# jstmn/cppflow

Hardware: AMD Instinct MI355X
Metric: LM-IK iterations/sec (seeds x waypoints) (higher is better)
Workload: dtype f32

## Files before the change

cppflow_amd/csrc/cppflow_hip.hip:

```cpp
#include <hip/hip_runtime.h>

#include <dlfcn.h>

#include <atomic>
#include <cmath>
#include <cstdio>
#include <cstring>
#include <mutex>
#include <new>
#include <string>
#include <type_traits>
#include <vector>

#include "../../include/cppflow_hip_debug.h"
#include "lmik_device.h"
#include "robots_gen.h"

using namespace cppf;

namespace cppf {
bool launch_fused_static(int static_id, int coll, unsigned grid, size_t lds, hipStream_t st, const FusedArgs& args);
int fused_static_block();
}

// ... 397 lines not shown
    if (const char* dump = std::getenv("CPPF_RTC_DUMP")) {
        std::ofstream f(dump);
        f << source;
    }
    uint64_t key = fnv1a(source);
    for (int i = 0; i < kEmbeddedCount; ++i) key = fnv1a(kEmbeddedSources[i], key);
    for (int i = 0; i < kRtcOptionCount; ++i) key = fnv1a(kRtcOptions[i], key);
    key = fnv1a(rtc_version_string(), key);
    char hex[32];
    std::snprintf(hex, sizeof hex, "%016llx", (unsigned long long)key);
    const std::string dir = rtc_cache_dir(cache_dir), file = dir + "/robot_" + hex + ".cppfrtc";
    std::vector<std::string> names;
    std::string code;
    if (!rtc_cache_read(dir, file, names, code)) {
        if (int rc = rtc_compile(source, with_quad, names, code)) return rc;
        rtc_cache_write(dir, file, names, code);
    }
    DeviceGuard device_guard__(robot->device);
    if (device_guard__.err != hipSuccess)
        return fail(CPPF_ERR_HIP, std::string("cppflow_hip: selecting the robot's device failed: ") + hipGetErrorString(device_guard__.err));
    RtcModule* m = new (std::nothrow) RtcModule();
    if (!m) return fail(CPPF_ERR_HIP, "cppflow_hip: out of host memory");
    hipError_t e = hipModuleLoadData(&m->module, code.data());
    for (int i = 0; e == hipSuccess && i < RTC_COUNT; ++i) {
        if (!with_quad && (i == RTC_QUAD0 || i == RTC_QUAD1)) continue;
        e = hipModuleGetFunction(&m->fn[i], m->module, names[(size_t)i].c_str());
    }
    if (e != hipSuccess) {
        if (m->module) (void)hipModuleUnload(m->module);
        delete m;
        return fail(CPPF_ERR_HIP, std::string("cppflow_hip: loading the specialised code object failed: ") + hipGetErrorString(e));
    }
    robot->rtc = m;
    return CPPF_OK;
}

int cppf_robot_ndof(const cppf_robot* robot) { return robot ? robot->desc.ndof : CPPF_ERR_INVALID; }

int cppf_debug_fused_single_offset(void) { return (int)__builtin_offsetof(FusedArgs, single); }

int cppf_debug_rtc_compile(const cppf_robot_desc* desc, const char* cache_dir) {
    cppf_robot* rb = nullptr;
    if (int rc = cppf_robot_create(desc, kNoDevice, &rb)) return rc;
    rb->static_id = -1;
    rb->device = kNoDevice;
    const int rc = cppf_robot_specialize(rb, cache_dir);
    delete rb;
    return rc;
}

int cppf_robot_specialization(const cppf_robot* robot) {
    if (!robot) return CPPF_ERR_INVALID;
    return robot->static_id >= 0 ? robot->static_id : (robot->rtc ? CPPF_SPECIALIZATION_RTC : -1);
}

int cppf_debug_set(cppf_robot* robot, int key, int value) {
    CPPF_REQUIRE(robot, "robot handle is NULL");
    CPPF_REQUIRE(key >= 0 && key < CPPF_TUNE_COUNT, "unknown tuning key");
    robot->tune[key].store(value == CPPF_TUNE_DEFAULT ? kTuneDefaults[key] : value, std::memory_order_relaxed);
    return CPPF_OK;
}

int cppf_debug_get(const cppf_robot* robot, int key, int* value) {
    CPPF_REQUIRE(robot && value, "robot / value is NULL");
    CPPF_REQUIRE(key >= 0 && key < CPPF_TUNE_COUNT, "unknown tuning key");
    *value = tune(robot, key);
    return CPPF_OK;
}

int cppf_set_obstacles(cppf_robot* robot, int n_obs, const float* cuboids, const float* Rt) {
    CPPF_REQUIRE(robot, "robot handle is NULL");
    CPPF_REQUIRE(n_obs >= 0 && n_obs <= CPPF_MAX_OBSTACLES, "n_obs out of range");
    CPPF_REQUIRE(n_obs == 0 || (cuboids && Rt), "cuboids / Rt is NULL");
    for (int o = 0; o < n_obs; ++o) {
        const float* R = Rt + o * 12;
        const float I[9] = {1, 0, 0, 0, 1, 0, 0, 0, 1};
        for (int k = 0; k < 9; ++k)
            CPPF_REQUIRE(std::fabs(R[k] - I[k]) < 1e-8f, "only axis-aligned cuboids are supported (R must be I)");
        for (int k = 0; k < 3; ++k) {
            CPPF_REQUIRE(cuboids[o * 6 + k] <= cuboids[o * 6 + 3 + k], "cuboid min corner > max corner");
            robot->coll.obs_lo[o][k] = R[9 + k] + cuboids[o * 6 + k];
            robot->coll.obs_hi[o][k] = R[9 + k] + cuboids[o * 6 + 3 + k];
        }
    }
    robot->coll.nobs = n_obs;
    return CPPF_OK;
}

int cppf_set_joint_limit_padding(cppf_robot* robot, const float* lo_padded, const float* hi_padded) {
    CPPF_REQUIRE(robot, "robot handle is NULL");
    if (!lo_padded || !hi_padded) {
        robot->coll.has_jl = 0;
        return CPPF_OK;
    }
    for (int j = 0; j < robot->desc.ndof; ++j) {
        robot->coll.jl_lo[j] = lo_padded[j];
        robot->coll.jl_hi[j] = hi_padded[j];
    }
    robot->coll.has_jl = 1;
    return CPPF_OK;
}

int cppf_forward_kinematics(const cppf_robot* robot, const float* x, int n, float* poses, void* stream) {
    CPPF_ENTER(robot);
    CPPF_REQUIRE(n >= 0, "n < 0");
    if (n == 0) return CPPF_OK;
    CPPF_REQUIRE(x && poses, "x / poses is NULL");
    hipStream_t st = (hipStream_t)stream;
    return for_ndof(robot->desc.ndof, [&](auto dof) {
        hipLaunchKernelGGL((fk_kernel<decltype(dof)::D>), dim3(grid_for(n)), dim3(kBlock), 0, st, robot->chain, robot->coll, n, x, poses);
        return check_launch();
    });
}

int cppf_jacobian(const cppf_robot* robot, const float* x, int n, float* J, void* stream) {
    CPPF_ENTER(robot);
    CPPF_REQUIRE(n >= 0, "n < 0");
    if (n == 0) return CPPF_OK;
    CPPF_REQUIRE(x && J, "x / J is NULL");
    hipStream_t st = (hipStream_t)stream;
    return for_ndof(robot->desc.ndof, [&](auto dof) {
        hipLaunchKernelGGL((jacobian_kernel<decltype(dof)::D>), dim3(grid_for(n)), dim3(kBlock), 0, st, robot->chain, robot->coll, n, x, J);
        return check_launch();
    });
}

int cppf_pose_errors(const cppf_robot* robot, const float* x, const float* target, int S, int W, float* e,
                     float* current_poses, void* stream) {
    CPPF_ENTER(robot);
    CPPF_REQUIRE(S >= 0 && W >= 0, "S / W < 0");
    const size_t n = (size_t)S * W;
    if (n == 0) return CPPF_OK;
    CPPF_REQUIRE(n <= 0x7fffffffu, "S*W exceeds 2^31-1 rows");
    CPPF_REQUIRE(x && target, "x / target is NULL");
    hipStream_t st = (hipStream_t)stream;
    return for_ndof(robot->desc.ndof, [&](auto dof) {
        hipLaunchKernelGGL((pose_errors_kernel<decltype(dof)::D>), dim3(grid_for(n)), dim3(kBlock), 0, st, robot->chain, robot->coll,
                           (int)n, W, x, target, e, current_poses);
        return check_launch();
    });
}

int cppf_clamp_to_joint_limits(const cppf_robot* robot, float* x, int n, void* stream) {
    CPPF_ENTER(robot);
    CPPF_REQUIRE(n >= 0, "n < 0");
    if (n == 0) return CPPF_OK;
    CPPF_REQUIRE(x, "x is NULL");
    const size_t total = (size_t)n * robot->desc.ndof;
    hipLaunchKernelGGL(clamp_kernel, dim3(grid_for(total)), dim3(kBlock), 0, (hipStream_t)stream, robot->chain, total, x);
    return check_launch();
}

}

namespace {

int make_lm_kernel_params(const cppf_robot* robot, const cppf_lm_params* params, LmK& prm) {
    CPPF_REQUIRE(params, "params is NULL");
    CPPF_REQUIRE(params->n_steps >= 1, "n_steps must be >= 1");
    CPPF_REQUIRE(params->clamp == 1 || params->n_steps == 1, "clamp = 0 is only defined for a single step");
    CPPF_REQUIRE(params->lm_lambda > 0.f, "lm_lambda must be > 0");
    CPPF_REQUIRE(params->alpha_position > 0.f && params->alpha_rotation > 0.f, "alpha_position / alpha_rotation must be > 0");
    CPPF_REQUIRE(params->solver == CPPF_SOLVER_AUTO || params->solver == CPPF_SOLVER_F32 || params->solver == CPPF_SOLVER_F64,
                 "unknown solver");
    CPPF_REQUIRE(params->solver_gate >= 0.f, "solver_gate must be >= 0 (0 = the default tolerance)");
    CPPF_REQUIRE(params->shape == CPPF_SHAPE_AUTO || params->shape == CPPF_SHAPE_ROW || params->shape == CPPF_SHAPE_QUAD,
// ... 1048 lines not shown
```

cppflow_amd/csrc/kernels_chain.h:

```cpp
#pragma once


template <int D>
__device__ __forceinline__ void load_x(const float* __restrict__ x, size_t row, float (&q)[D]) {
    const float* p = x + row * D;
    if constexpr (D % 4 == 0) {
#pragma unroll
        for (int k = 0; k < D / 4; ++k) {
            const float4 v = reinterpret_cast<const float4*>(p)[k];
            q[4 * k] = v.x, q[4 * k + 1] = v.y, q[4 * k + 2] = v.z, q[4 * k + 3] = v.w;
        }
    } else {
#pragma unroll
        for (int j = 0; j < D; ++j) q[j] = p[j];
    }
}

template <int D>
__device__ __forceinline__ void store_x(float* __restrict__ x, size_t row, const float (&q)[D]) {
    float* p = x + row * D;
    if constexpr (D % 4 == 0) {
#pragma unroll
        for (int k = 0; k < D / 4; ++k)
            reinterpret_cast<float4*>(p)[k] = make_float4(q[4 * k], q[4 * k + 1], q[4 * k + 2], q[4 * k + 3]);
// ... 86 lines not shown
}

#ifndef CPPF_LEAN_TRIG
#define CPPF_LEAN_TRIG 1
#endif
#ifndef CPPF_LEAN_RPY_FAST
#define CPPF_LEAN_RPY_FAST 1
#endif
__device__ __forceinline__ float atan_lean_poly(float a) {
    const float s = a * a;
    float p = 0.007374001666903496f;
    p = CPPF_FMA(p, s, -0.03551986813545227f);
    p = CPPF_FMA(p, s, 0.08216774463653564f);
    p = CPPF_FMA(p, s, -0.13398799300193787f);
    p = CPPF_FMA(p, s, 0.1986185610294342f);
    p = CPPF_FMA(p, s, -0.3332539498806f);
    return CPPF_FMA(a * s, p, a);
}
__device__ __forceinline__ float atan_lean_fixup(float a, float ax, float ay, float x, float y) {
    float r = atan_lean_poly(a);
    r = ay > ax ? 1.57079632679489661923f - r : r;
    r = x < 0.f ? 3.14159265358979323846f - r : r;
    return __builtin_copysignf(r, y);
}
__device__ __forceinline__ void atan2_pair_lean(float y1, float x1, float y2, float x2, float& r1, float& r2) {
    const float ax1 = fabsf(x1), ay1 = fabsf(y1), ax2 = fabsf(x2), ay2 = fabsf(y2);
    const float mx1 = fmaxf(fmaxf(ax1, ay1), 1e-15f), mx2 = fmaxf(fmaxf(ax2, ay2), 1e-15f);
    const float inv = __builtin_amdgcn_rcpf(mx1 * mx2);
    r1 = atan_lean_fixup(fminf(ax1, ay1) * (inv * mx2), ax1, ay1, x1, y1);
    r2 = atan_lean_fixup(fminf(ax2, ay2) * (inv * mx1), ax2, ay2, x2, y2);
}
__device__ __forceinline__ float asin_lean(float x) {
    const float ax = fabsf(x);
    const bool big = ax > 0.5f;

    const float z = big ? CPPF_FMA(-0.5f, ax, 0.5f) : x * x;
    const float t = big ? __builtin_amdgcn_sqrtf(z) : ax;
    float p = 0.05158697068691254f;
    p = CPPF_FMA(p, z, 0.03919339179992676f);
    p = CPPF_FMA(p, z, 0.07554031163454056f);
    p = CPPF_FMA(p, z, 0.16664926707744598f);
    float r = CPPF_FMA(t * z, p, t);
    r = big ? CPPF_FMA(-2.f, r, 1.57079632679489661923f) : r;
    return __builtin_copysignf(r, x);
}

template <bool LEAN = false>
__device__ __forceinline__ void pose_error(const float (&Rt)[9], const float (&tt)[3], const float (&R)[9],
                                           const float (&p)[3], float (&e)[6]) {
    const float e20 = dot3(Rt[6], Rt[7], Rt[8], R[0], R[1], R[2]);
    const float e21 = dot3(Rt[6], Rt[7], Rt[8], R[3], R[4], R[5]);
    const float e22 = dot3(Rt[6], Rt[7], Rt[8], R[6], R[7], R[8]);
    const float e10 = dot3(Rt[3], Rt[4], Rt[5], R[0], R[1], R[2]);
    const float e00 = dot3(Rt[0], Rt[1], Rt[2], R[0], R[1], R[2]);
    float sp = -e20;
    sp = sp > 1.f ? 1.f : (sp < -1.f ? -1.f : sp);
    if constexpr (LEAN && CPPF_LEAN_TRIG != 0) {
        const bool general = !(fabsf(sp) <= 0.5f) | !(fabsf(e21) <= e22) | !(fabsf(e10) <= e00);
        if (CPPF_LEAN_RPY_FAST != 0 && __builtin_expect(__builtin_amdgcn_ballot_w64(general) == 0ull, 1)) {
            const float inv = __builtin_amdgcn_rcpf(e22 * e00);
            const float a1 = e21 * (inv * e00), a2 = e10 * (inv * e22);
            e[0] = atan_lean_poly(a1);
            e[2] = atan_lean_poly(a2);
            const float z = sp * sp;
            float p = 0.05158697068691254f;
            p = CPPF_FMA(p, z, 0.03919339179992676f);
            p = CPPF_FMA(p, z, 0.07554031163454056f);
            p = CPPF_FMA(p, z, 0.16664926707744598f);
            e[1] = CPPF_FMA(sp * z, p, sp);
        } else {
            atan2_pair_lean(e21, e22, e10, e00, e[0], e[2]);
            e[1] = asin_lean(sp);
        }
    } else {
        e[0] = atan2_lm(e21, e22);
        e[1] = asin_lm(sp);
        e[2] = atan2_lm(e10, e00);
    }
    e[3] = tt[0] - p[0];
    e[4] = tt[1] - p[1];
    e[5] = tt[2] - p[2];
}

__device__ __forceinline__ void pose_metrics(const float (&Rt)[9], const float (&tt)[3], const float (&R)[9],
                                             const float (&p)[3], float& pos_err, float& rot_err) {
    const float dx = tt[0] - p[0], dy = tt[1] - p[1], dz = tt[2] - p[2];
    pos_err = __builtin_sqrtf(CPPF_FMA(dz, dz, CPPF_FMA(dy, dy, dx * dx)));
    float E[9];
#pragma unroll
    for (int i = 0; i < 3; ++i)
#pragma unroll
        for (int j = 0; j < 3; ++j)
            E[3 * i + j] = dot3(Rt[3 * i], Rt[3 * i + 1], Rt[3 * i + 2], R[3 * j], R[3 * j + 1], R[3 * j + 2]);
    const float a0 = E[7] - E[5], a1 = E[2] - E[6], a2 = E[3] - E[1];
    const float sn = 0.5f * __builtin_sqrtf(CPPF_FMA(a2, a2, CPPF_FMA(a1, a1, a0 * a0)));
    const float cs = 0.5f * (E[0] + E[4] + E[8] - 1.f);
    const float theta = atan2f(sn, cs);
    rot_err = fmaxf(theta, 8.94427191e-4f);
}

template <int D>
__device__ __forceinline__ void lm_dual_solve_y(const float (&J)[6][D], const float (&e)[6], float lam_r, float lam_p,
                                                float (&y)[6], float& est) {
    float L[6][6], inv[6], dmax = 0.f;
#pragma unroll
    for (int j = 0; j < 6; ++j) {
        const float lam = j < 3 ? lam_r : lam_p;
#pragma unroll
        for (int i = j; i < 6; ++i) {
            float s = (i == j) ? lam : 0.f;
#pragma unroll
            for (int k = 0; k < D; ++k) s = cfma2(J[i][k], J[j][k], s);
            if (i == j) dmax = fmaxf(dmax, s);
#pragma unroll
            for (int k = 0; k < j; ++k) s = CPPF_FMA(-L[i][k], L[j][k], s);
            if (i == j) {
                s = fmaxf(s, lam);
                inv[j] = __builtin_amdgcn_rsqf(s);
            } else {
                L[i][j] = s * inv[j];
            }
        }
    }
#pragma unroll
    for (int i = 0; i < 6; ++i) {
        float s = e[i];
#pragma unroll
        for (int k = 0; k < i; ++k) s = CPPF_FMA(-L[i][k], y[k], s);
        y[i] = s * inv[i];
    }
#pragma unroll
    for (int i = 5; i >= 0; --i) {
        float s = y[i];
#pragma unroll
        for (int k = i + 1; k < 6; ++k) s = CPPF_FMA(-L[k][i], y[k], s);
        y[i] = s * inv[i];
    }
    est = dmax * fmaxf(fmaxf(fmaxf(fabsf(y[0]), fabsf(y[1])), fmaxf(fabsf(y[2]), fabsf(y[3]))), fmaxf(fabsf(y[4]), fabsf(y[5])));
}

#ifndef CPPF_LEAN_BLOCK_SOLVE
#define CPPF_LEAN_BLOCK_SOLVE 1
#endif
template <int D>
__device__ __forceinline__ void lm_dual_solve_y_blk(const float (&J)[6][D], const float (&e)[6], float lam_r, float lam_p,
                                                    float (&y)[6], float& est) {
    float A[6][6], dmax = 0.f;
#pragma unroll
    for (int i = 0; i < 6; ++i)
#pragma unroll
        for (int j = 0; j <= i; ++j) {
            float s = (i == j) ? (i < 3 ? lam_r : lam_p) : 0.f;
#pragma unroll
            for (int k = 0; k < D; ++k) s = cfma2(J[i][k], J[j][k], s);
            A[i][j] = s;
            if (i == j) dmax = fmaxf(dmax, s);
        }
    float w0[6][3], w1[6][3], ia[3], ib[3], ic[3];
#pragma unroll
    for (int k = 0; k < 3; ++k) {
        const int p = 2 * k;
        const float a = A[p][p], b = A[p + 1][p], c = A[p + 1][p + 1];
        const float det = fmaxf(CPPF_FMA(a, c, -(b * b)), (p + 1 < 3 ? lam_r : lam_p) * a);
        const float r = __builtin_amdgcn_rcpf(det);
        ia[k] = c * r, ib[k] = -(b * r), ic[k] = a * r;
#pragma unroll
        for (int i = p + 2; i < 6; ++i) {
            w0[i][k] = CPPF_FMA(A[i][p + 1], ib[k], A[i][p] * ia[k]);
            w1[i][k] = CPPF_FMA(A[i][p + 1], ic[k], A[i][p] * ib[k]);
        }
#pragma unroll
        for (int i = p + 2; i < 6; ++i)
#pragma unroll
            for (int j = p + 2; j <= i; ++j) A[i][j] = CPPF_FMA(-w1[i][k], A[j][p + 1], CPPF_FMA(-w0[i][k], A[j][p], A[i][j]));
    }
    float u[6];
#pragma unroll
    for (int i = 0; i < 6; ++i) u[i] = e[i];
#pragma unroll
    for (int k = 0; k < 3; ++k) {
        const int p = 2 * k;
// ... 288 lines not shown
```

cppflow_amd/csrc/kernels_collision.h:

```cpp
#pragma once

struct CollOut {
    float min_self, min_env;
    int self_hit, env_hit;
};

__device__ __forceinline__ bool cull_far(float lower2, float cull2) {
    return __builtin_amdgcn_ballot_w64(!(lower2 > cull2)) == 0ull;
}

__device__ __forceinline__ float mid_dist2(const float (&a)[3], const float (&b)[3]) {
    const float dx = a[0] - b[0], dy = a[1] - b[1], dz = a[2] - b[2];
    return CPPF_FMA(dz, dz, CPPF_FMA(dy, dy, dx * dx));
}

__device__ __forceinline__ float point_box_dist2(const float (&m)[3], const float* __restrict__ lo,
                                                 const float* __restrict__ hi) {
    const float ex = m[0] - clampf(m[0], lo[0], hi[0]), ey = m[1] - clampf(m[1], lo[1], hi[1]),
                ez = m[2] - clampf(m[2], lo[2], hi[2]);
    return CPPF_FMA(ez, ez, CPPF_FMA(ey, ey, ex * ex));
}

template <class RB>
__device__ __forceinline__ void fk_capsules_to_lds(const RB& rb, const CollK& co, const float (&q)[RB::D],
                                                   float* __restrict__ lds, int tid, float (&R)[9], float (&p)[3]) {
    frame_identity(R, p);
    for (int c = co.cap_begin[0]; c < co.cap_begin[1]; ++c) {
#pragma unroll
        for (int k = 0; k < 3; ++k) {
            lds[(c * 6 + k) * kBlock + tid] = co.cap_c[c][k];
            lds[(c * 6 + 3 + k) * kBlock + tid] = co.cap_h[c][k];
        }
    }
#pragma unroll
    for (int j = 0; j < RB::D; ++j) {
        fk_fixed_joint(rb, j, R, p);
        fk_joint(R, p, rb.pris(j), q[j]);
        for (int c = co.cap_begin[j + 1]; c < co.cap_begin[j + 2]; ++c) {
            float wc[3], wh[3];
            xform_point(R, p, co.cap_c[c][0], co.cap_c[c][1], co.cap_c[c][2], wc);
            xform_dir(R, co.cap_h[c][0], co.cap_h[c][1], co.cap_h[c][2], wh);
#pragma unroll
            for (int k = 0; k < 3; ++k) {
                lds[(c * 6 + k) * kBlock + tid] = wc[k];
                lds[(c * 6 + 3 + k) * kBlock + tid] = wh[k];
            }
        }
    }
}

template <class RB>
__device__ __forceinline__ void capsule_fk_static(const RB& rb, const float (&q)[RB::D], float (&R)[9], float (&p)[3],
                                                  float (&wc)[(RB::Table::L > 0 ? RB::Table::L : 1)][3],
                                                  float (&wh)[(RB::Table::L > 0 ? RB::Table::L : 1)][3]) {
    using T = typename RB::Table;
    frame_identity(R, p);
#pragma unroll
    for (int c = 0; c < T::L; ++c) {
        if (T::cap_link[c] < 0) {
#pragma unroll
            for (int k = 0; k < 3; ++k) {
                wc[c][k] = T::cap_c[c][k];
                wh[c][k] = T::cap_h[c][k];
            }
        }
    }
#pragma unroll
    for (int j = 0; j < RB::D; ++j) {
        fk_fixed_joint(rb, j, R, p);
        fk_joint(R, p, rb.pris(j), q[j]);
#pragma unroll
        for (int c = 0; c < T::L; ++c) {
            if (T::cap_link[c] == j) {
                xform_point(R, p, T::cap_c[c][0], T::cap_c[c][1], T::cap_c[c][2], wc[c]);
                xform_dir(R, T::cap_h[c][0], T::cap_h[c][1], T::cap_h[c][2], wh[c]);
            }
        }
    }
}

__device__ __forceinline__ uint32_t cuboids_in_reach(const CollK& co, const float (&c)[3], float cull2) {
    uint32_t near = 0u;
    for (int o = 0; o < co.nobs; ++o)
        if (!cull_far(point_box_dist2(c, co.obs_lo[o], co.obs_hi[o]), cull2)) near |= 1u << o;
    return near;
}

template <class RB, bool WANT_MIN>
__device__ __forceinline__ CollOut collide_tests_static(const CollK& co,
                                                        const float (&wc)[(RB::Table::L > 0 ? RB::Table::L : 1)][3],
                                                        const float (&wh)[(RB::Table::L > 0 ? RB::Table::L : 1)][3],
                                                        bool do_self, bool do_env) {
    using T = typename RB::Table;
    CollOut r;
    r.min_self = INFINITY;
    r.self_hit = 0;
    if (do_self) {
#pragma unroll
        for (int pi = 0; pi < T::P; ++pi) {
            const int a = T::pair_a[pi], b = T::pair_b[pi];
            if constexpr (!WANT_MIN) {
                if (cull_far(mid_dist2(wc[a], wc[b]), T::pair_cull[pi])) continue;
            }
            const float d2 = seg_seg_dist2(wc[a], wh[a], wc[b], wh[b], T::cap_a[a], T::cap_ia[a], T::cap_a[b], T::cap_ia[b]);
            if constexpr (WANT_MIN) {
                const float v = __builtin_sqrtf(d2) - (T::cap_r[a] + T::cap_r[b]);
                r.min_self = v < r.min_self ? v : r.min_self;
            } else {
                r.self_hit |= d2 < T::pair_thr[pi];
            }
        }
    }
    if constexpr (WANT_MIN) r.self_hit = r.min_self < 0.f;
    r.min_env = INFINITY;
    r.env_hit = 0;
    if (do_env) {
#pragma unroll
        for (int c = 0; c < T::L; ++c) {
            uint32_t near = ~0u;
            if constexpr (!WANT_MIN) {
                near = cuboids_in_reach(co, wc[c], T::cap_cull[c]);
                if (near == 0u) continue;
            }
            for (int o = 0; o < co.nobs; ++o) {
                if (!((near >> o) & 1u)) continue;
                const float d2 = seg_box_dist2(wc[c], wh[c], co.obs_lo[o], co.obs_hi[o]);
                if constexpr (WANT_MIN) {
                    const float v = __builtin_sqrtf(d2) - T::cap_r[c];
                    r.min_env = v < r.min_env ? v : r.min_env;
                } else {
                    r.env_hit |= d2 < T::cap_thr[c];
                }
            }
        }
        if constexpr (WANT_MIN) r.env_hit = r.min_env < 0.f;
    }
    return r;
}

__device__ __forceinline__ void lds_capsule(const float* __restrict__ lds, int tid, int c, float (&wc)[3], float (&wh)[3]) {
#pragma unroll
    for (int k = 0; k < 3; ++k) {
        wc[k] = lds[(c * 6 + k) * kBlock + tid];
        wh[k] = lds[(c * 6 + 3 + k) * kBlock + tid];
    }
}

template <bool WANT_MIN>
__device__ __forceinline__ CollOut collide_from_lds(const CollK& co, const float* __restrict__ lds, int tid,
                                                    bool do_self, bool do_env) {
    CollOut r;
    r.min_self = INFINITY;
    r.self_hit = 0;
    if (do_self) {
        for (int pi = 0; pi < co.npairs; ++pi) {
            const int a = co.pair_a[pi], b = co.pair_b[pi];
            float ca[3], ha[3], cb[3], hb[3];
            lds_capsule(lds, tid, a, ca, ha);
            lds_capsule(lds, tid, b, cb, hb);
            if constexpr (!WANT_MIN) {
                if (cull_far(mid_dist2(ca, cb), co.pair_cull[pi])) continue;
            }
            const float d2 = seg_seg_dist2(ca, ha, cb, hb, co.cap_a[a], co.cap_ia[a], co.cap_a[b], co.cap_ia[b]);
            if constexpr (WANT_MIN) {
// ... 70 lines not shown
```

cppflow_amd/csrc/kernels_fused.h:

```cpp
#pragma once


__device__ __forceinline__ void load_target(const float* __restrict__ target, int w, float (&Rt)[9], float (&tt)[3]) {
    const float* t = target + (size_t)w * 7;
    tt[0] = t[0], tt[1] = t[1], tt[2] = t[2];
    quat_to_mat(t[3], t[4], t[5], t[6], Rt);
}

struct RowSummary {
    float pos_err = 0.f, rot_err = 0.f, cost = 0.f;
    int self_hit = 0, env_hit = 0, jl = 0;
};

template <int CTRL>
__device__ __forceinline__ float dpp_or_zero(float x) {
    return __builtin_bit_cast(float, __builtin_amdgcn_update_dpp(0, __builtin_bit_cast(int, x), CTRL, 0xf, 0xf, false));
}

template <bool IS_MAX>
__device__ __forceinline__ float wave_reduce_to_lane63(float v) {
    auto op = [](float a, float b) { return IS_MAX ? fmaxf(a, b) : a + b; };
    const float s1 = dpp_or_zero<0x111>(v), s2 = dpp_or_zero<0x112>(v), s3 = dpp_or_zero<0x113>(v);
    v = op(op(v, s1), op(s2, s3));
    v = op(v, dpp_or_zero<0x114>(v));
    v = op(v, dpp_or_zero<0x118>(v));
    v = op(v, dpp_or_zero<0x142>(v));
    v = op(v, dpp_or_zero<0x143>(v));
    return v;
}

__device__ __forceinline__ void lds_barrier() { asm volatile("s_waitcnt lgkmcnt(0)\n\ts_barrier" ::: "memory"); }

template <class RB>
__device__ __forceinline__ void block_seed_summary(const RB& rb, int W, size_t row, bool active, const float (&q)[RB::D],
                                                   const RowSummary& rs, float* __restrict__ out) {
    constexpr int D = RB::D;
    __shared__ float s_q[kBlock / 64][D];
    __shared__ float s_red[kBlock / 64][8];
    const int tid = threadIdx.x, lane = tid & 63, wave = tid >> 6;
    const float rad2deg = 57.29577951308232087680f;
    const int wps = W >> 6;
    if (wps > 1) {
        if (lane == 0) {
#pragma unroll
            for (int j = 0; j < D; ++j) s_q[wave][j] = q[j];
        }
        lds_barrier();
    }
    const bool seed_ends_here = ((wave + 1) & (wps - 1)) == 0;
    const bool has_next = active && !(lane == 63 && seed_ends_here);
    const int nw = wave + 1 < kBlock / 64 ? wave + 1 : wave;
    float mrev = 0.f, mpri = 0.f;
    float dq[D], wr[D];
#pragma unroll
    for (int j = 0; j < D; ++j) {
        float qn = dpp_or_zero<0x130>(q[j]);
        qn = (lane == 63) ? s_q[nw][j] : qn;
        dq[j] = wr[j] = qn - q[j];
    }
    wrap_pi_all<D>(wr);
#pragma unroll
    for (int j = 0; j < D; ++j) {
        const bool pr = rb.pris(j);
        const float a = nan_to_inf(pr ? fabsf(100.f * dq[j]) : fabsf(rad2deg * wr[j]));
        mpri = fmaxf(mpri, pr ? a : 0.f);
        mrev = fmaxf(mrev, pr ? 0.f : a);
    }
    float v[8] = {nan_to_inf(100.f * rs.pos_err), nan_to_inf(rad2deg * rs.rot_err), has_next ? mrev : 0.f, has_next ? mpri : 0.f,
                  (float)rs.self_hit, (float)rs.env_hit, (float)rs.jl, rs.cost};
#pragma unroll
    for (int k = 0; k < 8; ++k) v[k] = active ? v[k] : 0.f;
#pragma unroll
    for (int k = 0; k < 4; ++k) v[k] = wave_reduce_to_lane63<true>(v[k]);
#pragma unroll
    for (int k = 4; k < 8; ++k) v[k] = wave_reduce_to_lane63<false>(v[k]);
    float* o = out + ((uint32_t)row >> (31 - __builtin_clz((uint32_t)W))) * 8;
    if (wps == 1) {
        if (active && lane == 63) {
#pragma unroll
            for (int k = 0; k < 8; ++k) o[k] = v[k];
        }
        return;
    }
    if (lane == 63) {
#pragma unroll
        for (int k = 0; k < 8; ++k) s_red[wave][k] = v[k];
    }
    lds_barrier();
    if (active && lane == 63 && seed_ends_here) {
        for (int i = 1; i < wps; ++i) {
#pragma unroll
            for (int k = 0; k < 4; ++k) v[k] = fmaxf(v[k], s_red[wave - i][k]);
#pragma unroll
            for (int k = 4; k < 8; ++k) v[k] += s_red[wave - i][k];
        }
#pragma unroll
        for (int k = 0; k < 8; ++k) o[k] = v[k];
    }
}

#ifndef CPPF_LM_PACE
#define CPPF_LM_PACE 1
#endif
__device__ __forceinline__ void lm_pace(uint32_t t0, int k, int pace) {
    if (CPPF_LM_PACE == 0 || pace == 0) return;
    const int lag = (int)((uint32_t)__builtin_amdgcn_s_memrealtime() - t0) - k * pace, half = pace >> 1;
    if (lag > half)
        __builtin_amdgcn_s_setprio(3);
    else if (lag > 0)
        __builtin_amdgcn_s_setprio(2);
    else if (lag > -half)
        __builtin_amdgcn_s_setprio(1);
    else
        __builtin_amdgcn_s_setprio(0);
}

template <class RB>
__device__ __forceinline__ void lm_row_load(int W, const float* __restrict__ x_in, const float* __restrict__ target,
                                            size_t row, float (&q)[RB::D], float (&Rt)[9], float (&tt)[3]) {
    load_x<RB::D>(x_in, row, q);
    load_target(target, (int)((uint32_t)row % (uint32_t)W), Rt, tt);
}

#ifndef CPPF_LEAD_SINCOS
#define CPPF_LEAD_SINCOS 2
#endif
#ifndef CPPF_FIRST_LEAN
#define CPPF_FIRST_LEAN 1
#endif
template <class RB, bool LEAD, bool FIRST = false>
constexpr int lead_sincos() {
    return LEAD ? (FIRST && CPPF_LEAD_SINCOS == 2 ? 3 : CPPF_LEAD_SINCOS) : 0;
}
template <class RB, bool LEAD, bool FIRST = false>
__device__ __forceinline__ bool lm_row_iterate(const RB& rb, const LmK& prm, const cppf_lm_outputs& out, size_t row, bool last,
                                               const float (&Rt)[9], const float (&tt)[3], float* __restrict__ gate_lds,
                                               float (&q)[RB::D]) {
    constexpr int D = RB::D;
    float delta[D];
    bool conv = false;
    {
        float R[9], p[3], ax[D][3], og[D][3], J[6][D], e[6];
        fk_ee_axes<RB, lead_sincos<RB, LEAD, FIRST>()>(rb, q, R, p, ax, og);
        pose_error<LEAD>(Rt, tt, R, p, e);
        if constexpr (!LEAD) {
            if (prm.tol_pos2 > 0.f) {
                conv = dot3(e[3], e[4], e[5], e[3], e[4], e[5]) < prm.tol_pos2 && dot3(e[0], e[1], e[2], e[0], e[1], e[2]) < prm.tol_rot2;
                if (__builtin_amdgcn_ballot_w64(!conv) == 0ull) return true;
            }
        }
        jacobian_from_axes<RB>(rb, p, ax, og, J);
        float est = 0.f;
        if constexpr (D < 6) {
            lm_primal_solve<D>(J, e, prm.lm_lambda, prm.a_pos, prm.a_rot, delta);
        } else {
            float y[6];
            if constexpr (LEAD && CPPF_LEAN_BLOCK_SOLVE != 0)
                lm_dual_solve_y_blk<D>(J, e, prm.lam_r, prm.lam_p, y, est);
// ... 27 lines not shown
                        cut |= (v < rb.lo(j)) | (v > rb.hi(j));
                    }
                    flag = flag && !cut;
                }
                if constexpr (LEAD) {
                    if (prm.gate_thr > -INFINITY) {
                        const float es2 = CPPF_FMA(prm.a_pos * prm.a_pos, dot3(e[3], e[4], e[5], e[3], e[4], e[5]),
                                                   prm.a_rot * prm.a_rot * dot3(e[0], e[1], e[2], e[0], e[1], e[2]));
                        flag = flag && est * est > prm.gate_rel2 * es2;
                    }
                }
                unsigned long long todo = __builtin_amdgcn_ballot_w64(flag);
                if (todo != 0ull) {
                    int rank = lm_gate_hand_over<D>(J, e, todo, gate_lds, flag);
                    lm_gate_solve<D>(prm.lam_r_d, prm.lam_p_d, todo, rank, gate_lds, flag, delta);
                    while ((todo = __builtin_amdgcn_ballot_w64(flag)) != 0ull) {
                        float R2[9], p2[3], ax2[D][3], og2[D][3], J2[6][D], e2[6];
#pragma unroll
                        for (int j = 0; j < D; ++j) asm volatile("" : "+v"(q[j]));
                        fk_ee_axes<RB, lead_sincos<RB, LEAD, FIRST>()>(rb, q, R2, p2, ax2, og2);
                        pose_error<LEAD>(Rt, tt, R2, p2, e2);
                        jacobian_from_axes<RB>(rb, p2, ax2, og2, J2);
                        rank = lm_gate_hand_over<D>(J2, e2, todo, gate_lds, flag);
                        lm_gate_solve<D>(prm.lam_r_d, prm.lam_p_d, todo, rank, gate_lds, flag, delta);
                    }
                }
            }
        }
    }
    if constexpr (!LEAD) {
        if (prm.tol_pos2 > 0.f) {
            if (!conv) {
#pragma unroll
                for (int j = 0; j < D; ++j) q[j] += delta[j];
                if (prm.clamp) clamp_row<RB>(rb, q);
            }
            return conv;
        }
    }
#pragma unroll
    for (int j = 0; j < D; ++j) q[j] += delta[j];
    if (prm.clamp) clamp_row<RB>(rb, q);
    return false;
}

template <class RB, int COLL>
__device__ __forceinline__ void lm_row_finish(const RB& rb, const CollK& co, const cppf_lm_outputs& out, float* lds, int tid,
                                              size_t row, const float (&Rt)[9], const float (&tt)[3], const float (&q)[RB::D],
                                              RowSummary& rs) {
    constexpr int D = RB::D;
    if (out.x_out) store_x<D>(out.x_out, row, q);
    const bool want_metrics = out.pos_err_m || out.rot_err_rad || out.seed_summary;
    if constexpr (COLL != 0) {
        const bool do_self = out.self_mask || out.min_self || out.ext_cost || out.seed_summary;
        const bool do_env = out.env_mask || out.min_env || out.ext_cost || out.seed_summary;
        rs.jl = jlim_hit<D>(co, q);
        CollOut c;
        auto metrics = [&](float (&R)[9], float (&p)[3]) {
            if (want_metrics) {
                fk_fixed_ee(rb, R, p);
                pose_metrics(Rt, tt, R, p, rs.pos_err, rs.rot_err);
                if (out.pos_err_m) out.pos_err_m[row] = rs.pos_err;
                if (out.rot_err_rad) out.rot_err_rad[row] = rs.rot_err;
            }
        };
        if constexpr (RB::kStatic) {
            constexpr int L = RB::Table::L > 0 ? RB::Table::L : 1;
            float wc[L][3], wh[L][3];
            {
                float R[9], p[3];
                capsule_fk_static<RB>(rb, q, R, p, wc, wh);
                metrics(R, p);
            }
            c = collide_tests_static<RB, COLL == 2>(co, wc, wh, do_self, do_env);
        } else {
            {
                float R[9], p[3];
                fk_capsules_to_lds<RB>(rb, co, q, lds, tid, R, p);
                metrics(R, p);
            }
            c = collide_from_lds<COLL == 2>(co, lds, tid, do_self, do_env);
        }
        rs.self_hit = c.self_hit, rs.env_hit = c.env_hit;
        rs.cost = 100.f * (float)rs.jl + 1000.f * (float)c.env_hit + 1000.f * (float)c.self_hit;
        write_coll_outputs(row, c, rs.jl, out.self_mask, out.env_mask, out.jlim_mask, out.ext_cost, out.min_self,
                           out.min_env);
    } else {
        if (want_metrics) {
            float R[9], p[3];
            fk_ee<RB>(rb, q, R, p);
            pose_metrics(Rt, tt, R, p, rs.pos_err, rs.rot_err);
            if (out.pos_err_m) out.pos_err_m[row] = rs.pos_err;
            if (out.rot_err_rad) out.rot_err_rad[row] = rs.rot_err;
        }
    }
}

template <class RB>
constexpr int lm_waves() {
    return RB::kStatic ? (RB::D <= 7 ? 4 : 3) : (RB::D <= 6 ? 4 : (RB::D <= 8 ? 3 : 2));
}

template <class T>
__device__ __forceinline__ T* as_global(T* p) {
    return (T*)(__attribute__((address_space(1))) T*)p;
}

typedef const __attribute__((address_space(4))) BatchItemK* BatchItemPtr;

__device__ __forceinline__ BatchItemPtr fused_item(const void* table, uint32_t& blk) {
    typedef const __attribute__((address_space(4))) char* CPtr;
    blk = blockIdx.x;
    BatchItemPtr itp = (BatchItemPtr)((CPtr)__builtin_amdgcn_kernarg_segment_ptr() + __builtin_offsetof(FusedArgs, single));
    if (table) {
        const CPtr tab = (CPtr)(uintptr_t)table;
        const __attribute__((address_space(4))) BatchHeadK* hd = (const __attribute__((address_space(4))) BatchHeadK*)tab;
        uint32_t b = 0, begin = 0;
#pragma unroll
        for (int i = 0; i < CPPF_MAX_BATCH - 1; ++i) {
            const uint32_t e = hd->block_end[i];
            const bool past = blk >= e;
            b = past ? (uint32_t)(i + 1) : b;
            begin = past ? e : begin;
        }
        blk -= begin;
        itp = (BatchItemPtr)(tab + sizeof(BatchHeadK)) + b;
    }
    return itp;
}

__device__ __forceinline__ cppf_lm_outputs fused_outputs(BatchItemPtr itp) {
    cppf_lm_outputs o;
    o.x_out = as_global(itp->out.x_out), o.J_out = as_global(itp->out.J_out), o.e_out = as_global(itp->out.e_out);
    o.pos_err_m = as_global(itp->out.pos_err_m), o.rot_err_rad = as_global(itp->out.rot_err_rad);
    o.self_mask = as_global(itp->out.self_mask), o.env_mask = as_global(itp->out.env_mask), o.jlim_mask = as_global(itp->out.jlim_mask);
    o.ext_cost = as_global(itp->out.ext_cost), o.min_self = as_global(itp->out.min_self), o.min_env = as_global(itp->out.min_env);
    o.seed_summary = as_global(itp->out.seed_summary), o.n_iters = as_global(itp->out.n_iters);
    return o;
}

template <class RB, int COLL>
__global__ __launch_bounds__(kBlock) __attribute__((amdgpu_waves_per_eu(lm_waves<RB>(), lm_waves<RB>()))) void lm_fused_kernel(const ChainK ch, const CollK co, const LmK prm,
                                                          const BatchItemK single, const void* table) {
    extern __shared__ float lds[];
    (void)single;
    constexpr int D = RB::D;
    __shared__ float s_gate[kBlock / 64][GateLds<D>::kFloats];
    static_assert(sizeof(s_gate) + (kBlock / 64) * (D + 8) * sizeof(float) <= fused_static_lds_bound(D), "fused_static_lds_bound is stale");
    const RB rb{ch, co};
    uint32_t blk;
    const BatchItemPtr itp = fused_item(table, blk);
    const cppf_lm_outputs out = fused_outputs(itp);
    const int tid = threadIdx.x;
    const size_t row = (size_t)(blk * (unsigned)kBlock + (unsigned)tid);
    const bool active = row < (size_t)itp->n;
    float q[D];
#pragma unroll
    for (int j = 0; j < D; ++j) q[j] = 0.f;
    RowSummary rs;
    if (active) {
        float Rt[9], tt[3];
        lm_row_load<RB>(itp->W, as_global(itp->x_in), as_global(itp->target), row, q, Rt, tt);
        float chk = tt[0] + tt[1] + tt[2];
#pragma unroll
        for (int j = 0; j < D; ++j) chk += q[j];
#pragma unroll
        for (int k = 0; k < 9; ++k) chk += Rt[k];
// ... 232 lines not shown
```

cppflow_amd/csrc/lmik_device.h:

```cpp
#pragma once

#include <hip/hip_runtime.h>
#ifndef __HIPCC_RTC__
#include <stdint.h>
#endif

#include "../../include/cppflow_hip.h"

#ifndef INFINITY
#define INFINITY __builtin_huge_valf()
#endif

#define CPPF_FMA(a, b, c) __builtin_fmaf((a), (b), (c))

namespace cppf {

struct ChainK {
    float F[CPPF_MAX_DOF][12];
    float Fee[12];
    float lo[CPPF_MAX_DOF];
    float hi[CPPF_MAX_DOF];
    uint32_t pris_mask;
    int32_t ndof;
};

struct CollK {
    float cap_c[CPPF_MAX_CAPSULES][3];
    float cap_h[CPPF_MAX_CAPSULES][3];
    float cap_a[CPPF_MAX_CAPSULES];
    float cap_ia[CPPF_MAX_CAPSULES];
    float cap_r[CPPF_MAX_CAPSULES];
    int32_t cap_begin[CPPF_MAX_DOF + 2];
    int8_t cap_link[CPPF_MAX_CAPSULES];
    float pair_thr[CPPF_MAX_PAIRS];
    float cap_thr[CPPF_MAX_CAPSULES];
    float pair_cull[CPPF_MAX_PAIRS];
    float cap_cull[CPPF_MAX_CAPSULES];
    uint8_t pair_a[CPPF_MAX_PAIRS];
    uint8_t pair_b[CPPF_MAX_PAIRS];
    float obs_lo[CPPF_MAX_OBSTACLES][3];
    float obs_hi[CPPF_MAX_OBSTACLES][3];
    float jl_lo[CPPF_MAX_DOF];
    float jl_hi[CPPF_MAX_DOF];
    int32_t ncaps, npairs, nobs, has_jl;
};

struct LmK {
    double lam_r_d, lam_p_d;
    float lam_r, lam_p;
    float lm_lambda, a_pos, a_rot;
    int32_t n_steps, clamp;
    int32_t n, W;
    float tol_pos2, tol_rot2;
    float gate_thr;
    float gate_rel2;
    int32_t pace_ticks;
};

struct StepGateK {
    const int32_t* ctl;
    int32_t per_traj;
    uint32_t mask;
};
__device__ __forceinline__ bool step_open(const StepGateK& g, int s) {
    if (g.ctl == nullptr) return true;
    return ((g.mask >> (uint32_t)g.ctl[(size_t)(s * g.per_traj) * 16]) & 1u) != 0u;
}

struct BatchItemK {
    const float* x_in;
    const float* target;
    cppf_lm_outputs out;
    int32_t n, W;
};

struct BatchHeadK {
    uint32_t block_end[CPPF_MAX_BATCH];
};

struct FusedArgs {
    ChainK ch;
    CollK co;
    LmK prm;
    BatchItemK single;
    const void* table;
};

__device__ __forceinline__ float cmul(float x, float c) {
    if (__builtin_constant_p(c)) {
        if (c == 0.f) return 0.f;
        if (c == 1.f) return x;
        if (c == -1.f) return -x;
    }
    return x * c;
}

__device__ __forceinline__ float cfma(float x, float c, float acc) {
    if (__builtin_constant_p(c)) {
        if (c == 0.f) return acc;
        if (__builtin_constant_p(acc) && acc == 0.f) return cmul(x, c);
        if (c == 1.f) return acc + x;
        if (c == -1.f) return acc - x;
    }
    return CPPF_FMA(x, c, acc);
}

__device__ __forceinline__ float cfma2(float a, float b, float acc) {
    if (__builtin_constant_p(a) && a == 0.f) return acc;
    return cfma(a, b, acc);
}

template <int D_>
struct DynRobot {
    static constexpr int D = D_;
    static constexpr bool kStatic = false;
    const ChainK& ch;
    const CollK& co;
    __device__ __forceinline__ float F(int j, int k) const { return ch.F[j][k]; }
    __device__ __forceinline__ float Fee(int k) const { return ch.Fee[k]; }
    __device__ __forceinline__ bool pris(int j) const { return (ch.pris_mask >> j) & 1u; }
    __device__ __forceinline__ float lo(int j) const { return ch.lo[j]; }
    __device__ __forceinline__ float hi(int j) const { return ch.hi[j]; }
};

// ... 346 lines not shown
```

Baseline: 79.38 billion.

## Add union-box obstacle cull, rotation-floor shortcut, and ballot-based summary counts

Adds a precomputed union bounding box of all obstacles so a wave can skip per-obstacle checks when every lane is far from the union. Skips atan2 in pose_metrics when the whole wave has a near-identity rotation error and returns the floor value directly. Replaces the float wave reductions for hit and joint-limit counts with ballot+popcount and derives cost from those counts, which drops the per-row cost field. These are three independent shortcuts in the metrics and collision epilogues; the rotation shortcut returns the floor for angles that may sit slightly above it.

Measured after the change: 80.45 billion (median of 6 runs). 1.3% higher.

```diff
diff --git a/cppflow_amd/csrc/cppflow_hip.hip b/cppflow_amd/csrc/cppflow_hip.hip
--- a/cppflow_amd/csrc/cppflow_hip.hip
+++ b/cppflow_amd/csrc/cppflow_hip.hip
@@ -503,6 +503,15 @@
             robot->coll.obs_lo[o][k] = R[9 + k] + cuboids[o * 6 + k];
             robot->coll.obs_hi[o][k] = R[9 + k] + cuboids[o * 6 + 3 + k];
         }
+    }
+    for (int k = 0; k < 3; ++k) {
+        float ulo = 0.f, uhi = 0.f;
+        for (int o = 0; o < n_obs; ++o) {
+            ulo = o == 0 ? robot->coll.obs_lo[o][k] : std::fmin(ulo, robot->coll.obs_lo[o][k]);
+            uhi = o == 0 ? robot->coll.obs_hi[o][k] : std::fmax(uhi, robot->coll.obs_hi[o][k]);
+        }
+        robot->coll.obs_ulo[k] = ulo;
+        robot->coll.obs_uhi[k] = uhi;
     }
     robot->coll.nobs = n_obs;
     return CPPF_OK;
diff --git a/cppflow_amd/csrc/kernels_chain.h b/cppflow_amd/csrc/kernels_chain.h
--- a/cppflow_amd/csrc/kernels_chain.h
+++ b/cppflow_amd/csrc/kernels_chain.h
@@ -192,6 +192,9 @@
     e[5] = tt[2] - p[2];
 }
 
+#ifndef CPPF_ROT_FLOOR_SHORTCUT
+#define CPPF_ROT_FLOOR_SHORTCUT 1
+#endif
 __device__ __forceinline__ void pose_metrics(const float (&Rt)[9], const float (&tt)[3], const float (&R)[9],
                                              const float (&p)[3], float& pos_err, float& rot_err) {
     const float dx = tt[0] - p[0], dy = tt[1] - p[1], dz = tt[2] - p[2];
@@ -205,8 +208,12 @@
     const float a0 = E[7] - E[5], a1 = E[2] - E[6], a2 = E[3] - E[1];
     const float sn = 0.5f * __builtin_sqrtf(CPPF_FMA(a2, a2, CPPF_FMA(a1, a1, a0 * a0)));
     const float cs = 0.5f * (E[0] + E[4] + E[8] - 1.f);
-    const float theta = atan2f(sn, cs);
-    rot_err = fmaxf(theta, 8.94427191e-4f);
+    const float floor_rad = 8.94427191e-4f;
+    if (CPPF_ROT_FLOOR_SHORTCUT != 0 && __builtin_amdgcn_ballot_w64(!(sn <= 4e-4f && cs >= 0.5f)) == 0ull) {
+        rot_err = floor_rad;
+        return;
+    }
+    rot_err = fmaxf(atan2f(sn, cs), floor_rad);
 }
 
 template <int D>
diff --git a/cppflow_amd/csrc/kernels_collision.h b/cppflow_amd/csrc/kernels_collision.h
--- a/cppflow_amd/csrc/kernels_collision.h
+++ b/cppflow_amd/csrc/kernels_collision.h
@@ -79,7 +79,13 @@
     }
 }
 
+#ifndef CPPF_UNION_BOX
+#define CPPF_UNION_BOX 1
+#endif
 __device__ __forceinline__ uint32_t cuboids_in_reach(const CollK& co, const float (&c)[3], float cull2) {
+    if (CPPF_UNION_BOX != 0 && co.nobs > 1) {
+        if (cull_far(point_box_dist2(c, co.obs_ulo, co.obs_uhi), cull2)) return 0u;
+    }
     uint32_t near = 0u;
     for (int o = 0; o < co.nobs; ++o)
         if (!cull_far(point_box_dist2(c, co.obs_lo[o], co.obs_hi[o]), cull2)) near |= 1u << o;
diff --git a/cppflow_amd/csrc/kernels_fused.h b/cppflow_amd/csrc/kernels_fused.h
--- a/cppflow_amd/csrc/kernels_fused.h
+++ b/cppflow_amd/csrc/kernels_fused.h
@@ -8,7 +8,7 @@
 }
 
 struct RowSummary {
-    float pos_err = 0.f, rot_err = 0.f, cost = 0.f;
+    float pos_err = 0.f, rot_err = 0.f;
     int self_hit = 0, env_hit = 0, jl = 0;
 };
 
@@ -29,6 +29,9 @@
     return v;
 }
 
+#ifndef CPPF_SUMMARY_BALLOT
+#define CPPF_SUMMARY_BALLOT 1
+#endif
 __device__ __forceinline__ void lds_barrier() { asm volatile("s_waitcnt lgkmcnt(0)\n\ts_barrier" ::: "memory"); }
 
 template <class RB>
@@ -67,13 +70,21 @@
         mrev = fmaxf(mrev, pr ? 0.f : a);
     }
     float v[8] = {nan_to_inf(100.f * rs.pos_err), nan_to_inf(rad2deg * rs.rot_err), has_next ? mrev : 0.f, has_next ? mpri : 0.f,
-                  (float)rs.self_hit, (float)rs.env_hit, (float)rs.jl, rs.cost};
-#pragma unroll
-    for (int k = 0; k < 8; ++k) v[k] = active ? v[k] : 0.f;
-#pragma unroll
-    for (int k = 0; k < 4; ++k) v[k] = wave_reduce_to_lane63<true>(v[k]);
-#pragma unroll
-    for (int k = 4; k < 8; ++k) v[k] = wave_reduce_to_lane63<false>(v[k]);
+                  0.f, 0.f, 0.f, 0.f};
+#pragma unroll
+    for (int k = 0; k < 4; ++k) v[k] = wave_reduce_to_lane63<true>(active ? v[k] : 0.f);
+    if constexpr (CPPF_SUMMARY_BALLOT != 0) {
+        const int n_self = __builtin_popcountll(__builtin_amdgcn_ballot_w64(active && rs.self_hit != 0));
+        const int n_env = __builtin_popcountll(__builtin_amdgcn_ballot_w64(active && rs.env_hit != 0));
+        const int n_jl = __builtin_popcountll(__builtin_amdgcn_ballot_w64(active && rs.jl != 0));
+        v[4] = (float)n_self, v[5] = (float)n_env, v[6] = (float)n_jl;
+        v[7] = (float)(100 * n_jl + 1000 * (n_env + n_self));
+    } else {
+        const float cost = 100.f * (float)rs.jl + 1000.f * (float)rs.env_hit + 1000.f * (float)rs.self_hit;
+        v[4] = (float)rs.self_hit, v[5] = (float)rs.env_hit, v[6] = (float)rs.jl, v[7] = cost;
+#pragma unroll
+        for (int k = 4; k < 8; ++k) v[k] = wave_reduce_to_lane63<false>(active ? v[k] : 0.f);
+    }
     float* o = out + ((uint32_t)row >> (31 - __builtin_clz((uint32_t)W))) * 8;
     if (wps == 1) {
         if (active && lane == 63) {
@@ -267,7 +278,6 @@
             c = collide_from_lds<COLL == 2>(co, lds, tid, do_self, do_env);
         }
         rs.self_hit = c.self_hit, rs.env_hit = c.env_hit;
-        rs.cost = 100.f * (float)rs.jl + 1000.f * (float)c.env_hit + 1000.f * (float)c.self_hit;
         write_coll_outputs(row, c, rs.jl, out.self_mask, out.env_mask, out.jlim_mask, out.ext_cost, out.min_self,
                            out.min_env);
     } else {
diff --git a/cppflow_amd/csrc/lmik_device.h b/cppflow_amd/csrc/lmik_device.h
--- a/cppflow_amd/csrc/lmik_device.h
+++ b/cppflow_amd/csrc/lmik_device.h
@@ -40,6 +40,8 @@
     uint8_t pair_b[CPPF_MAX_PAIRS];
     float obs_lo[CPPF_MAX_OBSTACLES][3];
     float obs_hi[CPPF_MAX_OBSTACLES][3];
+    float obs_ulo[3];
+    float obs_uhi[3];
     float jl_lo[CPPF_MAX_DOF];
     float jl_hi[CPPF_MAX_DOF];
     int32_t ncaps, npairs, nobs, has_jl;
```
